# AntreasAntoniou/HowToTrainYourMAMLPytorch

Measured on AMD Instinct MI355X. Metric: meta-tasks/sec, higher is better.
Workload: dtype bf16; 1 GPU; model=maml++_miniimagenet_5w1s, global_batch=128, tasks_per_gpu=128, ways=5, shots=1, targets=15, filters=48, inner_steps=5, msl=True, parallelism=task-dp1

## Files before the change

howtotrainyourmamlpytorch_amd/ops/hip/conv_host.h:

```cpp
#pragma once

#include <cstdlib>
#include <vector>

#include <hip/hip_bf16.h>
#include <torch/extension.h>

namespace maml355 {

inline bool deterministic_mode() {
  const char* e = getenv("MAML355_DETERMINISTIC");
  return e && e[0] == '1';
}

inline int wgrad_nsub_override() {
  const char* e = getenv("MAML355_WGRAD_NSUB");
  return e && (e[0] == '1' || e[0] == '2') ? e[0] - '0' : 0;
}

const __hip_bfloat16* conv_zero_page(const torch::Tensor& like);

std::vector<torch::Tensor> finish_wgrad(const torch::Tensor& acc,
                                        const torch::Tensor& dbacc, int T,
                                        int F, int C, int nslices,
                                        hipStream_t stream);

}
```

howtotrainyourmamlpytorch_amd/ops/hip/tconv.hip:

```cpp

#include "common.h"
#include "conv_host.h"
#include "tconv_mm_addr.h"
#include "wgrad_plan.h"
#include <torch/extension.h>
#include <ATen/cuda/CUDAContext.h>

using namespace maml355;

using bf16 = __hip_bfloat16;
typedef __attribute__((__vector_size__(8 * sizeof(short)))) short bf16x8;
typedef __attribute__((__vector_size__(4 * sizeof(float)))) float f32x4;

DEVINL int swz64(int row, int col) {
  return (row * 64 + col) ^ ((row & 7) << 3);
}
DEVINL int swz128(int row, int col) {
  return (row * 128 + col) ^ ((row & 7) << 3);
}

__global__ void repack_weight_kernel(const float* __restrict__ w,
                                     bf16* __restrict__ wp,
                                     int T, int F, int C, bool dgrad) {
  const long total = (long)T * F * C * 9;
  for (long i = (long)blockIdx.x * blockDim.x + threadIdx.x; i < total;
       i += grid_stride()) {
    long r = i;
    const int kx = (int)(r % 3); r /= 3;
    const int ky = (int)(r % 3); r /= 3;
    const int c = (int)(r % C); r /= C;
    const int f = (int)(r % F); r /= F;
    const long t = r;
    const float v = w[i];
    long o;
    if (!dgrad) {
      o = (((t * 9 + (long)(ky * 3 + kx)) * C + c) * F) + f;
    } else {
      o = (((t * 9 + (long)((2 - ky) * 3 + (2 - kx))) * F + f) * C) + c;
    }
    wp[o] = __float2bfloat16(v);
  }
}

__global__ void wgrad_finalize_kernel(const float* __restrict__ acc,
                                      float* __restrict__ dw,
                                      int T, int F, int C, int nslices) {
  const long total = (long)T * F * C * 9;
  const long ssz = (long)9 * C * F;
  for (long i = (long)blockIdx.x * blockDim.x + threadIdx.x; i < total;
       i += grid_stride()) {
    long r = i;
    const int kx = (int)(r % 3); r /= 3;
    const int ky = (int)(r % 3); r /= 3;
    const int c = (int)(r % C); r /= C;
    const int f = (int)(r % F); r /= F;
    const long t = r;
    const long e = ((long)(ky * 3 + kx) * C + c) * F + f;
    float v = 0.f;
    for (int s = 0; s < nslices; ++s) {
      v += acc[(t * nslices + s) * ssz + e];
    }
    dw[i] = v;
  }
}

#define BM 256
#define BK 64
#define WBK 64

#define WGN 64
static_assert(WBK == wgplan::kStep && WGN == wgplan::kCols,
              "wgrad_plan.h cuts K-chunks for these tiles");

__global__ __launch_bounds__(512, 2)
void tconv_mm_kernel(const bf16* __restrict__ X, const bf16* __restrict__ Wp,
                     const float* __restrict__ bias, bf16* __restrict__ Y,
                     float* __restrict__ sums_out,
                     int T, int NB, int H, int W, int Ci,
                     int Ho, int Wo, int Co, int pad) {
  const int t = blockIdx.y;
  const long Mtot = (long)NB * Ho * Wo;
  const long m0 = (long)blockIdx.x * BM;
  const int K9 = 9 * Ci;
  const int ksteps = (K9 + BK - 1) / BK;
  const int ntiles = (Co + 15) / 16;

  __shared__ short lds_a[BM * BK];
  __shared__ short lds_bt[64 * BK];
  __shared__ int row_h[BM], row_w[BM], row_n[BM];
  __shared__ int ktab_dy[576 + BK], ktab_dx[576 + BK], ktab_c[576 + BK];

  for (int m = threadIdx.x; m < BM; m += blockDim.x) {
    const long mg = m0 + m;
    if (mg < Mtot) {
      const int wo = (int)(mg % Wo);
      const int ho = (int)((mg / Wo) % Ho);
      const int n = (int)(mg / ((long)Wo * Ho));
      row_h[m] = ho; row_w[m] = wo; row_n[m] = n;
    } else {
      row_n[m] = -1;
    }
  }
  for (int k = threadIdx.x; k < ksteps * BK; k += blockDim.x) {
    if (k < K9) {
      const int kyx = k / Ci;
      ktab_c[k] = k - kyx * Ci;
      ktab_dy[k] = kyx / 3;
      ktab_dx[k] = kyx % 3;
    } else {
      ktab_c[k] = -1;
    }
  }

  const bf16* Xt = X + (long)t * NB * H * W * Ci;
  const bf16* Wt = Wp + (long)t * 9 * Ci * Co;

  const int wave = threadIdx.x / WAVE;
  const int lane = threadIdx.x % WAVE;
  const int fr = lane & 15;
  const int fk = lane >> 4;

  f32x4 acc[2][4];
#pragma unroll
  for (int hh = 0; hh < 2; ++hh)
#pragma unroll
    for (int i = 0; i < 4; ++i) acc[hh][i] = {0.f, 0.f, 0.f, 0.f};

  __syncthreads();
  for (int ks = 0; ks < ksteps; ++ks) {
    const int k0 = ks * BK;
    for (int s = threadIdx.x; s < BM * (BK / 8); s += blockDim.x) {
      const int m = s / (BK / 8);
      const int kk0 = (s % (BK / 8)) * 8;
      const int n = row_n[m];
      const int c0 = ktab_c[k0 + kk0];
      const int c7 = ktab_c[k0 + kk0 + 7];
      if ((Ci % 8 == 0) && c0 >= 0 && c7 == c0 + 7) {
        bf16x8 v = {0, 0, 0, 0, 0, 0, 0, 0};
        if (n >= 0) {
          const int h = row_h[m] + ktab_dy[k0 + kk0] - pad;
          const int w = row_w[m] + ktab_dx[k0 + kk0] - pad;
          if (h >= 0 && h < H && w >= 0 && w < W) {
            v = *(const bf16x8*)&(
                (const short*)Xt)[(((long)n * H + h) * W + w) * Ci + c0];
          }
        }
        *(bf16x8*)&lds_a[swz64(m, kk0)] = v;
      } else {
        for (int j = 0; j < 8; ++j) {
          const int kk = kk0 + j;
          const int c = ktab_c[k0 + kk];
          short v = 0;
          if (n >= 0 && c >= 0) {
            const int h = row_h[m] + ktab_dy[k0 + kk] - pad;
            const int w = row_w[m] + ktab_dx[k0 + kk] - pad;
            if (h >= 0 && h < H && w >= 0 && w < W) {
              v = ((const short*)Xt)[(((long)n * H + h) * W + w) * Ci + c];
            }
          }
          lds_a[swz64(m, kk & ~7) + (kk & 7)] = v;
        }
      }
    }
    for (int s = threadIdx.x; s < BK * 8; s += blockDim.x) {
      const int kk = s >> 3;
      const int f0 = (s & 7) * 8;
      if ((Co % 8 == 0) && f0 + 8 <= Co) {
        bf16x8 v = {0, 0, 0, 0, 0, 0, 0, 0};
        if (k0 + kk < K9) {
          v = *(const bf16x8*)&((const short*)Wt)[(long)(k0 + kk) * Co + f0];
        }
#pragma unroll
        for (int j = 0; j < 8; ++j)
          lds_bt[swz64(f0 + j, kk & ~7) + (kk & 7)] = v[j];
      } else {
        for (int j = 0; j < 8 && f0 + j < 64; ++j) {
          const int f = f0 + j;
          short v = 0;
          if (f < Co && k0 + kk < K9) {
            v = ((const short*)Wt)[(long)(k0 + kk) * Co + f];
          }
          lds_bt[swz64(f, kk & ~7) + (kk & 7)] = v;
        }
      }
    }
    __syncthreads();

#pragma unroll
    for (int ksl = 0; ksl < BK / 32; ++ksl) {
      bf16x8 a0 = *(const bf16x8*)&lds_a[swz64(wave * 32 + fr, ksl * 32 + fk * 8)];
      bf16x8 a1 = *(const bf16x8*)&lds_a[swz64(wave * 32 + 16 + fr, ksl * 32 + fk * 8)];
#pragma unroll
      for (int nt = 0; nt < 4; ++nt) {
        if (nt < ntiles) {
          bf16x8 b = *(const bf16x8*)&lds_bt[swz64(nt * 16 + fr, ksl * 32 + fk * 8)];
          acc[0][nt] = __builtin_amdgcn_mfma_f32_16x16x32_bf16(a0, b, acc[0][nt], 0, 0, 0);
          acc[1][nt] = __builtin_amdgcn_mfma_f32_16x16x32_bf16(a1, b, acc[1][nt], 0, 0, 0);
        }
      }
    }
    __syncthreads();
  }

  __shared__ float sums_lds[2][64];
  if (sums_out) {
    for (int i = threadIdx.x; i < 128; i += blockDim.x) {
      sums_lds[i >> 6][i & 63] = 0.f;
    }
    __syncthreads();
  }
  bf16* Yt = Y + (long)t * Mtot * Co;
#pragma unroll
  for (int hh = 0; hh < 2; ++hh)
#pragma unroll
  for (int nt = 0; nt < 4; ++nt) {
    if (nt >= ntiles) break;
    const int col = nt * 16 + fr;
    if (col >= Co) continue;
    const float bv = bias ? bias[(long)t * Co + col] : 0.f;
    float ls = 0.f, lq = 0.f;
#pragma unroll
    for (int j = 0; j < 4; ++j) {
      const int row = wave * 32 + hh * 16 + fk * 4 + j;
      const long mg = m0 + row;
      if (mg < Mtot) {
        const float v = acc[hh][nt][j] + bv;
        ((short*)Yt)[mg * Co + col] =
            (short)__bfloat16_as_short(__float2bfloat16(v));
        ls += v;
        lq += v * v;
      }
    }
    if (sums_out) {
      atomicAdd(&sums_lds[0][col], ls);
      atomicAdd(&sums_lds[1][col], lq);
    }
  }
  if (sums_out) {
    __syncthreads();
    for (int c = threadIdx.x; c < Co; c += blockDim.x) {
      atomicAdd(&sums_out[((long)t * 2 + 0) * Co + c], sums_lds[0][c]);
      atomicAdd(&sums_out[((long)t * 2 + 1) * Co + c], sums_lds[1][c]);
    }
  }
}

#define V2_LDS_BYTES (2 * BM * BK * 2 + 2 * 64 * BK * 2)
#define V2_LDS_BYTES_SBUF (BM * BK * 2 + 64 * BK * 2)

template <bool DBUF>
__global__ __launch_bounds__(512, 2)
void tconv_mm_v2_kernel(const bf16* __restrict__ X, const bf16* __restrict__ Wimg,
                        const float* __restrict__ bias, const bf16* __restrict__ zpage,
                        bf16* __restrict__ Y, float* __restrict__ sums_out,
                        int T, int NB, int H, int W, int Ci,
                        int Ho, int Wo, int Co, int pad) {
  const int t = blockIdx.y;
  const tcmm::Geom g = tcmm::make_geom(NB, H, W, Ci, Ho, Wo, pad);
  const long Mtot = g.Mtot;
  const long m0 = (long)blockIdx.x * BM;
  const int K9 = 9 * Ci;
  const int ksteps = (K9 + BK - 1) / BK;
  const int ntiles = (Co + 15) / 16;

  extern __shared__ short smem[];
#define LDS_A(buf_) (smem + (DBUF ? (buf_) * (BM * BK) : 0))
#define LDS_B(buf_) \
  (smem + (DBUF ? 2 : 1) * (BM * BK) + (DBUF ? (buf_) * (64 * BK) : 0))

  const bf16* Xt = X + (long)t * NB * H * W * Ci;
  const short* Wt = (const short*)Wimg + (long)t * ksteps * 64 * BK;

  const int wave = threadIdx.x / WAVE;
  const int lane = threadIdx.x % WAVE;
  const int fr = lane & 15;
  const int fk = lane >> 4;

  tcmm::KState a_k = tcmm::k_init(g, tcmm::slot_k8(threadIdx.x));
  tcmm::Row a_row[4];
#pragma unroll
  for (int q = 0; q < 4; ++q) {
    a_row[q] = tcmm::row_init(g, m0 + tcmm::slot_row(q * 512 + threadIdx.x));
  }
#define V2_ADVANCE() tcmm::k_advance(g, a_k)

#define V2_STAGE(ks_, buf_)                                                    \
  do {                                                                         \
    _Pragma("unroll")                                                          \
    for (int q = 0; q < 4; ++q) {                                              \
      int off;                                                                 \
      const bf16* src = tcmm::slot_src(g, a_row[q], a_k, off) ? Xt + off       \
                                                              : zpage;         \
      auto ldst = (__attribute__((address_space(3))) void*)(                   \
          &LDS_A(buf_)[((long)q * 512 + wave * 64) * 8]);                      \
      __builtin_amdgcn_global_load_lds(                                        \
          (const __attribute__((address_space(1))) void*)src, ldst, 16, 0, 0); \
    }                                                                          \
    {                                                                          \
      const short* bsrc = Wt + (long)(ks_)*64 * BK + (long)threadIdx.x * 8;    \
      auto ldst = (__attribute__((address_space(3))) void*)(                   \
          &LDS_B(buf_)[(long)wave * 64 * 8]);                                  \
      __builtin_amdgcn_global_load_lds(                                        \
          (const __attribute__((address_space(1))) void*)bsrc, ldst, 16, 0, 0);\
    }                                                                          \
  } while (0)

  f32x4 acc[2][4];
#pragma unroll
  for (int hh = 0; hh < 2; ++hh)
#pragma unroll
    for (int i = 0; i < 4; ++i) acc[hh][i] = {0.f, 0.f, 0.f, 0.f};

  int buf = 0;
  if (DBUF) {
    V2_STAGE(0, 0);
    __syncthreads();
  }
  for (int ks = 0; ks < ksteps; ++ks) {
    if (DBUF) {
      V2_ADVANCE();
      if (ks + 1 < ksteps) V2_STAGE(ks + 1, buf ^ 1);
    } else {
      V2_STAGE(ks, 0);
      V2_ADVANCE();
      __syncthreads();
    }
    const short* la = LDS_A(buf);
    const short* lb = LDS_B(buf);
#pragma unroll
    for (int ksl = 0; ksl < BK / 32; ++ksl) {
      bf16x8 a0 = *(const bf16x8*)&la[swz64(wave * 32 + fr, ksl * 32 + fk * 8)];
      bf16x8 a1 = *(const bf16x8*)&la[swz64(wave * 32 + 16 + fr, ksl * 32 + fk * 8)];
#pragma unroll
      for (int nt = 0; nt < 4; ++nt) {
        if (nt < ntiles) {
          bf16x8 b = *(const bf16x8*)&lb[swz64(nt * 16 + fr, ksl * 32 + fk * 8)];
          acc[0][nt] = __builtin_amdgcn_mfma_f32_16x16x32_bf16(a0, b, acc[0][nt], 0, 0, 0);
          acc[1][nt] = __builtin_amdgcn_mfma_f32_16x16x32_bf16(a1, b, acc[1][nt], 0, 0, 0);
        }
      }
    }
    __syncthreads();
    if (DBUF) buf ^= 1;
  }
#undef V2_STAGE
#undef V2_ADVANCE

  __shared__ float sums_lds[2][64];
  if (sums_out) {
    for (int i = threadIdx.x; i < 128; i += blockDim.x) {
      sums_lds[i >> 6][i & 63] = 0.f;
    }
    __syncthreads();
  }
  bf16* Yt = Y + (long)t * Mtot * Co;
#pragma unroll
  for (int hh = 0; hh < 2; ++hh)
#pragma unroll
  for (int nt = 0; nt < 4; ++nt) {
    if (nt >= ntiles) break;
    const int col = nt * 16 + fr;
    if (col >= Co) continue;
    const float bv = bias ? bias[(long)t * Co + col] : 0.f;
    float ls = 0.f, lq = 0.f;
#pragma unroll
    for (int j = 0; j < 4; ++j) {
      const int row = wave * 32 + hh * 16 + fk * 4 + j;
      const long mg = m0 + row;
      if (mg < Mtot) {
        const float v = acc[hh][nt][j] + bv;
        ((short*)Yt)[mg * Co + col] =
            (short)__bfloat16_as_short(__float2bfloat16(v));
        ls += v;
        lq += v * v;
      }
    }
    if (sums_out) {
      atomicAdd(&sums_lds[0][col], ls);
      atomicAdd(&sums_lds[1][col], lq);
    }
  }
  if (sums_out) {
    __syncthreads();
    for (int c = threadIdx.x; c < Co; c += blockDim.x) {
      atomicAdd(&sums_out[((long)t * 2 + 0) * Co + c], sums_lds[0][c]);
      atomicAdd(&sums_out[((long)t * 2 + 1) * Co + c], sums_lds[1][c]);
    }
  }
}

#undef LDS_A
#undef LDS_B

__global__ void pad_nhwc_kernel(const bf16* __restrict__ x, bf16* __restrict__ xp,
                                int T, int NB, int H, int W, int C, int pad) {
  const int Hp = H + 2 * pad, Wp = W + 2 * pad;
  const int c8n = C / 8;
  const long total = (long)T * NB * Hp * Wp * c8n;
  typedef bf16x8 v8;
  for (long i = (long)blockIdx.x * blockDim.x + threadIdx.x; i < total;
       i += grid_stride()) {
    const int c0 = (int)(i % c8n) * 8;
    long r = i / c8n;
    const int wp = (int)(r % Wp); r /= Wp;
    const int hp = (int)(r % Hp); r /= Hp;
    const long nb = r;
    const int h = hp - pad, w = wp - pad;
    v8 v = {0, 0, 0, 0, 0, 0, 0, 0};
    if (h >= 0 && h < H && w >= 0 && w < W) {
      v = *(const v8*)&((const short*)x)[((nb * H + h) * W + w) * C + c0];
    }
    *(v8*)&((short*)xp)[((nb * Hp + hp) * Wp + wp) * C + c0] = v;
  }
}

__global__ void repack_v2_kernel(const float* __restrict__ w,
                                 bf16* __restrict__ out,
                                 int T, int F, int C, int ksteps, bool dgrad) {
  const int cin = dgrad ? F : C;
  const int cout = dgrad ? C : F;
  const int K9 = 9 * cin;
  const long total = (long)T * ksteps * 64 * BK;
  for (long i = (long)blockIdx.x * blockDim.x + threadIdx.x; i < total;
       i += grid_stride()) {
    const int jj = (int)(i & 7);
    const int j = (int)((i >> 3) & 7);
    const int f = (int)((i >> 6) & 63);
    long r = i >> 12;
    const int ks = (int)(r % ksteps);
    const long t = r / ksteps;
    const int k = ks * BK + ((j ^ (f & 7)) * 8) + jj;
    float v = 0.f;
    if (k < K9 && f < cout) {
      const int kyx = k / cin;
      const int ci = k - kyx * cin;
      const int ky = kyx / 3, kx = kyx % 3;
      if (!dgrad) {
        v = w[((((long)t * F + f) * C + ci) * 3 + ky) * 3 + kx];
      } else {
        v = w[((((long)t * F + ci) * C + f) * 3 + (2 - ky)) * 3 + (2 - kx)];
      }
    }
    out[i] = __float2bfloat16(v);
  }
}


__global__ void dyt_pad_kernel(const bf16* __restrict__ dy,
                               bf16* __restrict__ dyt,
                               int T, int NB, int Ho, int Wo, int F,
                               int Wo8, long Kr) {
  __shared__ short lds[64 * 72];
  long b = blockIdx.x;
  const int ho = (int)(b % Ho); b /= Ho;
  const int n = (int)(b % NB); b /= NB;
  const int t = (int)b;
  const int f8n = (F + 7) / 8;
  const short* src = (const short*)dy + ((((long)t * NB + n) * Ho + ho) * Wo) * F;
  const long k0 = ((long)n * Ho + ho) * Wo8;
  short* dst = (short*)dyt + (long)t * F * Kr + k0;
  for (int wbase = 0; wbase < Wo8; wbase += 64) {
    const int wlen = min(64, Wo8 - wbase);
    for (int s = threadIdx.x; s < wlen * f8n; s += blockDim.x) {
      const int wl = s / f8n;
      const int wo = wbase + wl;
      const int f0 = (s % f8n) * 8;
      bf16x8 v = {0, 0, 0, 0, 0, 0, 0, 0};
      if (wo < Wo && f0 + 8 <= F) {
        v = *(const bf16x8*)&src[(long)wo * F + f0];
      } else if (wo < Wo) {
        for (int j = 0; j < 8 && f0 + j < F; ++j)
          v[j] = src[(long)wo * F + f0 + j];
      }
#pragma unroll
      for (int j = 0; j < 8; ++j) lds[(f0 + j) * 72 + wl] = v[j];
    }
    __syncthreads();
    for (int s = threadIdx.x; s < F * (wlen / 8); s += blockDim.x) {
      const int f = s / (wlen / 8);
      const int w0 = (s % (wlen / 8)) * 8;
      *(bf16x8*)&dst[(long)f * Kr + wbase + w0] =
          *(const bf16x8*)&lds[f * 72 + w0];
    }
    __syncthreads();
  }
}

__global__ void dyt_tail_kernel(bf16* __restrict__ dyt, int T, int F,
                                long Kprime, long Kr) {
  const long tail = Kr - Kprime;
  const long total = (long)T * F * tail;
  for (long i = (long)blockIdx.x * blockDim.x + threadIdx.x; i < total;
       i += grid_stride()) {
    const long c = i % tail;
    const long r = i / tail;
    ((short*)dyt)[r * Kr + Kprime + c] = 0;
  }
}

__global__ void xt_pad_kernel(const bf16* __restrict__ x, bf16* __restrict__ xt,
                              int T, int NB, int H, int W, int C,
                              int Hxp, int Wxp, int pad) {
  __shared__ short lds[64 * 72];
  long b = blockIdx.x;
  const int wt = (int)(b % ((Wxp + 63) / 64)); b /= (Wxp + 63) / 64;
  const int hxp = (int)(b % Hxp); b /= Hxp;
  const int n = (int)(b % NB); b /= NB;
  const int t = (int)b;
  const int h = hxp - pad;
  const int w0 = wt * 64;
  const int c8n = (C + 7) / 8;
  const short* src = (const short*)x + (((long)t * NB + n) * H) * W * C;
  for (int s = threadIdx.x; s < 64 * c8n; s += blockDim.x) {
    const int wl = s / c8n;
    const int c0 = (s % c8n) * 8;
    const int w = w0 + wl - pad;
    bf16x8 v = {0, 0, 0, 0, 0, 0, 0, 0};
    if (h >= 0 && h < H && w >= 0 && w < W) {
      if (c0 + 8 <= C) {
        v = *(const bf16x8*)&src[((long)h * W + w) * C + c0];
      } else {
        for (int j = 0; j < 8 && c0 + j < C; ++j)
          v[j] = src[((long)h * W + w) * C + c0 + j];
      }
    }
#pragma unroll
    for (int j = 0; j < 8; ++j) lds[(c0 + j) * 72 + wl] = v[j];
  }
  __syncthreads();
  short* dst = (short*)xt + ((((long)t * C) * NB + n) * Hxp + hxp) * Wxp;
  for (int s = threadIdx.x; s < C * 8; s += blockDim.x) {
    const int c = s / 8;
    const int wg = (s % 8) * 8;
    const int wx = w0 + wg;
    if (wx + 8 <= Wxp) {
      *(bf16x8*)&dst[((long)c * NB * Hxp) * Wxp + wx] =
          *(const bf16x8*)&lds[c * 72 + wg];
    } else {
      for (int j = 0; j < 8 && wx + j < Wxp; ++j)
        dst[((long)c * NB * Hxp) * Wxp + wx + j] = lds[c * 72 + wg + j];
    }
  }
}

template <int NSUB, bool DET>
__global__ __launch_bounds__(256, 4)
void tconv_wgrad_v2_kernel(const bf16* __restrict__ dYT,
                           const bf16* __restrict__ XT,
                           const bf16* __restrict__ zpage,
                           float* __restrict__ dWacc,
                           float* __restrict__ dBacc,
                           int T, int NB, int Ho, int Wo8, int Hxp, int Wxp,
                           int C, int F, long Kr, long Kprime, int kchunk) {
  const int t = blockIdx.z;
  const int n0 = blockIdx.x * (64 * NSUB);
  const int N9 = 9 * C;
  const long kc0 = (long)blockIdx.y * kchunk;
  const long kc_end = min(kc0 + (long)kchunk, Kr);
  const int mtiles = (F + 15) / 16;
  const long imgS = (long)NB * Hxp * Wxp;

  __shared__ short lds_at[2][64 * WBK];
  __shared__ short lds_bt[2][64 * NSUB * WBK];

  const bf16* dYTt = dYT + (long)t * F * Kr;
  const bf16* XTt = XT + (long)t * C * imgS;

  const int wave = threadIdx.x / WAVE;
  const int lane = threadIdx.x % WAVE;
  const int fr = lane & 15;
  const int fk = lane >> 4;

  int a_f[2], a_k8[2];
#pragma unroll
  for (int q = 0; q < 2; ++q) {
    const int s = q * 256 + threadIdx.x;
    a_f[q] = s >> 3;
    a_k8[q] = ((s & 7) ^ ((s >> 3) & 7)) * 8;
  }
  long b_imgoff[2 * NSUB];
  int b_wo8[2 * NSUB], b_ho[2 * NSUB];
  long b_k[2 * NSUB];
  bool b_valid[2 * NSUB];
#pragma unroll
  for (int q = 0; q < 2 * NSUB; ++q) {
    const int s = q * 256 + threadIdx.x;
    const int n = s >> 3;
    const int ng = n0 + n;
    b_valid[q] = ng < N9;
    const int kyx = b_valid[q] ? ng / C : 0;
    const int c = ng - kyx * C;
    b_k[q] = kc0 + ((s & 7) ^ (n & 7)) * 8;
    const int wo8 = (int)(b_k[q] % Wo8);
    const long line = b_k[q] / Wo8;
    const int ho = (int)(line % Ho);
    const int nimg = (int)(line / Ho);
    b_wo8[q] = wo8;
    b_ho[q] = ho;
    b_imgoff[q] = ((long)c * NB + nimg) * Hxp * Wxp +
                  (long)(ho + kyx / 3) * Wxp + kyx % 3;
  }

#define WG2_STAGE(k0_, buf_)                                                   \
  do {                                                                         \
    _Pragma("unroll")                                                          \
    for (int q = 0; q < 2; ++q) {                                              \
      const bf16* src = (a_f[q] < F)                                           \
                            ? dYTt + (long)a_f[q] * Kr + (k0_) + a_k8[q]       \
                            : zpage;                                           \
      auto ldst = (__attribute__((address_space(3))) void*)(                   \
          &lds_at[buf_][((long)q * 256 + wave * 64) * 8]);                     \
      __builtin_amdgcn_global_load_lds(                                        \
          (const __attribute__((address_space(1))) void*)src, ldst, 16, 0, 0); \
    }                                                                          \
    _Pragma("unroll")                                                          \
    for (int q = 0; q < 2 * NSUB; ++q) {                                       \
      const bf16* src = (b_valid[q] && b_k[q] < Kprime)                        \
                            ? XTt + b_imgoff[q] + b_wo8[q]                     \
                            : zpage;                                           \
      auto ldst = (__attribute__((address_space(3))) void*)(                   \
          &lds_bt[buf_][((long)q * 256 + wave * 64) * 8]);                     \
      __builtin_amdgcn_global_load_lds(                                        \
          (const __attribute__((address_space(1))) void*)src, ldst, 16, 0, 0); \
    }                                                                          \
  } while (0)

#define WG2_ADVANCE()                                                          \
  do {                                                                         \
    _Pragma("unroll")                                                          \
    for (int q = 0; q < 2 * NSUB; ++q) {                                       \
      b_k[q] += WBK;                                                           \
      b_wo8[q] += WBK;                                                         \
      while (b_wo8[q] >= Wo8) {                                                \
        b_wo8[q] -= Wo8;                                                       \
        ++b_ho[q];                                                             \
        b_imgoff[q] += Wxp;                                                    \
        if (b_ho[q] == Ho) {                                                   \
          b_ho[q] = 0;                                                         \
          b_imgoff[q] += (long)(Hxp - Ho) * Wxp;                               \
        }                                                                      \
      }                                                                        \
    }                                                                          \
  } while (0)

  f32x4 acc[NSUB][4];
#pragma unroll
  for (int sb = 0; sb < NSUB; ++sb)
#pragma unroll
// ... 543 lines not shown
```

howtotrainyourmamlpytorch_amd/ops/hip/wgrad_nt.hip:

```cpp

#include "common.h"
#include "conv_host.h"
#include "wgrad_nt_addr.h"
#include "wgrad_plan.h"
#include <torch/extension.h>
#include <ATen/cuda/CUDAContext.h>

using namespace maml355;

using bf16 = __hip_bfloat16;
typedef __attribute__((__vector_size__(8 * sizeof(short)))) short bf16x8;
typedef __attribute__((__vector_size__(4 * sizeof(float)))) float f32x4;
typedef short bf16x4v __attribute__((ext_vector_type(4)));

static_assert(wgnt::kRows == wgplan::kStep,
              "wgrad_plan.h cuts K-chunks for this tile");

enum {
  NT_BIAS_NONE = wgplan::kBiasNone,
  NT_BIAS_ONES = wgplan::kBiasOnes,
  NT_BIAS_COLSUM = wgplan::kBiasColsum
};

__global__ void nt_chpad8_kernel(const bf16* __restrict__ x,
                                 bf16* __restrict__ xp, long M, int C) {
  for (long i = (long)blockIdx.x * blockDim.x + threadIdx.x; i < M;
       i += grid_stride()) {
    bf16x8 v = {0, 0, 0, 0, 0, 0, 0, 0};
    const short* s = (const short*)x + i * C;
#pragma unroll
    for (int j = 0; j < 8; ++j)
      if (j < C) v[j] = s[j];
    *(bf16x8*)((short*)xp + i * 8) = v;
  }
}

DEVINL bf16x4v lds_read_tr(const short* p) {
  return __builtin_amdgcn_ds_read_tr16_b64_v4i16(
      (__attribute__((address_space(3))) bf16x4v*)p);
}

template <int NSUB, int MT, bool DET>
__global__ __launch_bounds__(256, 4)
void tconv_wgrad_nt_kernel(const bf16* __restrict__ dY,
                           const bf16* __restrict__ X,
                           const bf16* __restrict__ zpage,
                           float* __restrict__ dWacc,
                           float* __restrict__ dBacc,
                           wgnt::Geom g, int Cout, long Kr, int kchunk,
                           int bias_mode) {
  const int t = blockIdx.z;
  const int n0 = blockIdx.x * (64 * NSUB);
  const int F = g.F;
  const long kc0 = (long)blockIdx.y * kchunk;
  const long kc_end = min(kc0 + (long)kchunk, Kr);

  __shared__ __attribute__((aligned(16))) short lds_a[2][64 * 64];
  __shared__ __attribute__((aligned(16))) short lds_b[2][NSUB][64 * 64];

  const bf16* dYt = dY + (long)t * g.NB * g.Ho * g.Wo * F;
  const bf16* Xt = X + (long)t * g.NB * g.H * g.W * g.C;

  const int wave = __builtin_amdgcn_readfirstlane(threadIdx.x / WAVE);
  const int lane = threadIdx.x % WAVE;
  const int fr = lane & 15;
  const int fk = lane >> 4;

  int s_ch[2];
  wgnt::Pos s_pos[2];
  long s_k[2];
  wgnt::Col s_col[2][NSUB];
#pragma unroll
  for (int q = 0; q < 2; ++q) {
    const int s = q * 256 + threadIdx.x;
    s_ch[q] = wgnt::slot_chunk(s);
    s_k[q] = kc0 + wgnt::slot_row(s);
    s_pos[q] = wgnt::pos_from_k(g, s_k[q]);
#pragma unroll
    for (int sb = 0; sb < NSUB; ++sb)
      s_col[q][sb] = wgnt::col_from_n(g, n0 + sb * 64 + s_ch[q] * 8);
  }

#define NT_LOAD(src_, dst_)                                                    \
  __builtin_amdgcn_global_load_lds(                                            \
      (const __attribute__((address_space(1))) void*)(src_),                   \
      (__attribute__((address_space(3))) void*)(dst_), 16, 0, 0)

#define NT_STAGE(buf_)                                                         \
  do {                                                                         \
    _Pragma("unroll")                                                          \
    for (int q = 0; q < 2; ++q) {                                              \
      const long ao = wgnt::a_src(g, s_pos[q], s_k[q], s_ch[q]);                         \
      const bf16* asrc = ao == wgnt::kZeroPage ? zpage : dYt + ao;             \
      NT_LOAD(asrc, &lds_a[buf_][(q * 256 + wave * 64) * 8]);                  \
      _Pragma("unroll")                                                        \
      for (int sb = 0; sb < NSUB; ++sb) {                                      \
        const long bo = wgnt::b_src(g, s_pos[q], s_k[q], s_col[q][sb]);        \
        const bf16* bsrc = bo == wgnt::kZeroPage ? zpage : Xt + bo;            \
        NT_LOAD(bsrc, &lds_b[buf_][sb][(q * 256 + wave * 64) * 8]);            \
      }                                                                        \
    }                                                                          \
  } while (0)

#define NT_ADVANCE()                                                           \
  do {                                                                         \
    _Pragma("unroll")                                                          \
    for (int q = 0; q < 2; ++q) {                                              \
      s_k[q] += wgnt::kRows;                                                   \
      wgnt::pos_advance(g, s_pos[q]);                                          \
    }                                                                          \
  } while (0)

  f32x4 acc[NSUB][MT];
#pragma unroll
  for (int sb = 0; sb < NSUB; ++sb)
#pragma unroll
    for (int i = 0; i < MT; ++i) acc[sb][i] = {0.f, 0.f, 0.f, 0.f};

  const int ones_col = (bias_mode == NT_BIAS_ONES) ? g.N9 : -1;
  const int ncols = g.N9 + (bias_mode == NT_BIAS_ONES ? 1 : 0);
  bool sb_active[NSUB], sb_ones[NSUB];
#pragma unroll
  for (int sb = 0; sb < NSUB; ++sb) {
    const int nsub0 = n0 + (sb * 4 + wave) * 16;
    sb_active[sb] = nsub0 < ncols;
    sb_ones[sb] = nsub0 + fr == ones_col;
  }
  const bool do_colsum = (bias_mode == NT_BIAS_COLSUM) && (blockIdx.x == 0);
  float db_acc = 0.f;
  const int db_f = threadIdx.x & 63;
  const int db_q = threadIdx.x >> 6;

  NT_STAGE(0);
  __syncthreads();
  int buf = 0;
  for (long k0 = kc0; k0 < kc_end; k0 += wgnt::kRows) {
    NT_ADVANCE();
    if (k0 + wgnt::kRows < kc_end) NT_STAGE(buf ^ 1);
    const short* la = lds_a[buf];
#pragma unroll
    for (int ks = 0; ks < 2; ++ks) {
      bf16x8 afrag[MT];
#pragma unroll
      for (int mt = 0; mt < MT; ++mt) {
        const bf16x4v a0 = lds_read_tr(la + wgnt::tr_idx(lane, ks, 0, mt));
        const bf16x4v a1 = lds_read_tr(la + wgnt::tr_idx(lane, ks, 1, mt));
        afrag[mt] = {a0[0], a0[1], a0[2], a0[3], a1[0], a1[1], a1[2], a1[3]};
      }
#pragma unroll
      for (int sb = 0; sb < NSUB; ++sb) {
        if (!sb_active[sb]) continue;
        const short* lb = lds_b[buf][sb];
        const bf16x4v b0 = lds_read_tr(lb + wgnt::tr_idx(lane, ks, 0, wave));
        const bf16x4v b1 = lds_read_tr(lb + wgnt::tr_idx(lane, ks, 1, wave));
        bf16x8 bfrag = {b0[0], b0[1], b0[2], b0[3], b1[0], b1[1], b1[2], b1[3]};
        if (sb_ones[sb]) {
          const short one = 0x3F80;
          bfrag = {one, one, one, one, one, one, one, one};
        }
#pragma unroll
        for (int mt = 0; mt < MT; ++mt)
          acc[sb][mt] = __builtin_amdgcn_mfma_f32_16x16x32_bf16(
              afrag[mt], bfrag, acc[sb][mt], 0, 0, 0);
      }
    }
    if (do_colsum && db_f < F) {
#pragma unroll
      for (int kk = db_q * 16; kk < db_q * 16 + 16; ++kk) {
        db_acc += __bfloat162float(__hip_bfloat16(__hip_bfloat16_raw{
            (unsigned short)la[wgnt::lds_idx(kk, db_f)]}));
      }
    }
    __syncthreads();
    buf ^= 1;
  }
#undef NT_STAGE
#undef NT_ADVANCE
#undef NT_LOAD

  if (do_colsum) {
    __shared__ float db_lds[4][64];
    db_lds[db_q][db_f] = db_acc;
    __syncthreads();
    if (db_q == 0 && db_f < F) {
      const float v = db_lds[0][db_f] + db_lds[1][db_f] + db_lds[2][db_f] +
                      db_lds[3][db_f];
      if (DET) {
        dBacc[((long)t * gridDim.y + blockIdx.y) * F + db_f] = v;
      } else {
        atomicAdd(&dBacc[(long)t * F + db_f], v);
      }
    }
  }

  const long sl = DET ? (long)t * gridDim.y + blockIdx.y : (long)t;
  float* dWt = dWacc + sl * 9 * Cout * F;
  float* dBt = dBacc ? dBacc + sl * F : nullptr;
#pragma unroll
  for (int sb = 0; sb < NSUB; ++sb) {
    const int n = n0 + (sb * 4 + wave) * 16 + fr;
    const int orow = wgnt::out_row(g, n, Cout);
    float* dst = nullptr;
    if (orow >= 0) dst = dWt + (long)orow * F;
    else if (n == ones_col) dst = dBt;
    if (dst == nullptr) continue;
#pragma unroll
    for (int mt = 0; mt < MT; ++mt) {
#pragma unroll
      for (int j = 0; j < 4; ++j) {
        const int f = mt * 16 + fk * 4 + j;
        if (f < F) {
          if (DET) {
            dst[f] = acc[sb][mt][j];
          } else {
            atomicAdd(&dst[f], acc[sb][mt][j]);
          }
        }
      }
    }
  }
}

std::vector<torch::Tensor> tconv_wgrad_v3(torch::Tensor dy, torch::Tensor x,
                                          long pad, bool with_bias) {
  TORCH_CHECK(dy.is_cuda() && x.is_cuda());
  TORCH_CHECK(dy.scalar_type() == torch::kBFloat16 &&
              x.scalar_type() == torch::kBFloat16);
  auto dyc = dy.contiguous();
  auto xc = x.contiguous();
  const int T = (int)x.size(0), NB = (int)x.size(1), H = (int)x.size(2),
            W = (int)x.size(3), C = (int)x.size(4);
  const int Ho = (int)dy.size(2), Wo = (int)dy.size(3), F = (int)dy.size(4);
  TORCH_CHECK(F % 8 == 0 && F <= 64, "wgrad_v3 needs F % 8 == 0, F <= 64");
  TORCH_CHECK(C % 8 == 0 || C == 1 || C == 3,
              "wgrad_v3 needs C % 8 == 0 or C in {1, 3}");
  TORCH_CHECK(dy.size(0) == T && dy.size(1) == NB &&
              Ho == H + 2 * pad - 2 && Wo == W + 2 * pad - 2 &&
              Ho >= 1 && Wo >= 1 && pad >= 0 && pad <= 2,
              "wgrad_v3: dy/x shapes do not match a 3x3 stride-1 conv");
  const bool det = deterministic_mode();
  auto stream = at::cuda::getCurrentCUDAStream();

  int Cp = C;
  if (C % 8 != 0) {
    Cp = 8;
    const long M = (long)T * NB * H * W;
    auto xp = torch::empty({T, NB, H, W, 8}, x.options());
    hipLaunchKernelGGL(nt_chpad8_kernel,
                       dim3((unsigned)std::min<long>((M + 255) / 256, 65536)),
                       dim3(256), 0,
                       stream.stream(),
                       reinterpret_cast<const bf16*>(xc.data_ptr()),
                       reinterpret_cast<bf16*>(xp.data_ptr()), M, C);
    xc = xp;
  }
  const char* v2_env = getenv("MAML355_WGRAD_V2");
  const wgplan::Plan p =
      wgplan::v3(T, NB, Ho, Wo, C, with_bias, det,
                 !(v2_env && v2_env[0] == '0'), wgrad_nsub_override());
  const wgnt::Geom g =
      wgnt::make_geom(NB, H, W, Cp, Ho, Wo, F, (int)pad, p.Wk);
  TORCH_CHECK(p.gridy <= 65535 && T <= 65535, "wgrad_v3: grid too large");
  auto fopt = x.options().dtype(torch::kFloat32);
  auto acc = torch::zeros({T, p.nslices, 9 * C, F}, fopt);
  auto dbacc = torch::zeros({T, p.nslices, F}, fopt);
  const bf16* zpage = conv_zero_page(x);
  dim3 grid((unsigned)p.gridx, (unsigned)p.gridy, T);
#define LAUNCH_NT(NS_, MT_, DET_)                                              \
  hipLaunchKernelGGL((tconv_wgrad_nt_kernel<NS_, MT_, DET_>), grid, dim3(256), \
                     0, stream.stream(),                                       \
                     reinterpret_cast<const bf16*>(dyc.data_ptr()),            \
                     reinterpret_cast<const bf16*>(xc.data_ptr()), zpage,      \
                     acc.data_ptr<float>(),                                    \
                     with_bias ? dbacc.data_ptr<float>() : nullptr, g, C,      \
                     p.Kr, p.kchunk, p.bias)
#define LAUNCH_NT_MT(NS_, DET_)                                                \
  switch ((F + 15) / 16) {                                                     \
    case 1: LAUNCH_NT(NS_, 1, DET_); break;                                    \
    case 2: LAUNCH_NT(NS_, 2, DET_); break;                                    \
    case 3: LAUNCH_NT(NS_, 3, DET_); break;                                    \
    default: LAUNCH_NT(NS_, 4, DET_); break;                                   \
  }
  if (p.nsub == 2) {
    if (det) LAUNCH_NT_MT(2, true) else LAUNCH_NT_MT(2, false)
  } else {
    if (det) LAUNCH_NT_MT(1, true) else LAUNCH_NT_MT(1, false)
  }
#undef LAUNCH_NT_MT
#undef LAUNCH_NT
  return finish_wgrad(acc, dbacc, T, F, C, p.nslices, stream.stream());
}
```

Before: 734.3 tasks/s.

## Pipeline LDS DMA with explicit vmcnt waits and single barrier per k-step

Replaces the compiler global_load_lds path with inline-asm LDS DMA that sets m0 explicitly, in both the double-buffered forward conv and the wgrad kernel. Each k-step now waits on vmcnt and takes one barrier at the top instead of two __syncthreads, and the wgrad LDS buffers are merged so the bias reduction scratch reuses buffer space. Launch bounds for NSUB=2 are relaxed to 3 blocks per CU. The aim is less barrier and waitcnt overhead, at the cost of hand-written asm and occupancy/register tradeoffs.

```diff
diff --git a/howtotrainyourmamlpytorch_amd/ops/hip/conv_host.h b/howtotrainyourmamlpytorch_amd/ops/hip/conv_host.h
--- a/howtotrainyourmamlpytorch_amd/ops/hip/conv_host.h
+++ b/howtotrainyourmamlpytorch_amd/ops/hip/conv_host.h
@@ -18,6 +18,11 @@
   return e && (e[0] == '1' || e[0] == '2') ? e[0] - '0' : 0;
 }
 
+inline bool wgrad_pipe_enabled() {
+  const char* e = getenv("MAML355_WGRAD_PIPE");
+  return !(e && e[0] == '0');
+}
+
 const __hip_bfloat16* conv_zero_page(const torch::Tensor& like);
 
 std::vector<torch::Tensor> finish_wgrad(const torch::Tensor& acc,
diff --git a/howtotrainyourmamlpytorch_amd/ops/hip/lds_dma.h b/howtotrainyourmamlpytorch_amd/ops/hip/lds_dma.h
--- /dev/null
+++ b/howtotrainyourmamlpytorch_amd/ops/hip/lds_dma.h
@@ -0,0 +1,38 @@
+#pragma once
+
+#include "common.h"
+
+namespace maml355 {
+
+typedef unsigned lds_ptr;
+
+DEVINL lds_ptr lds_addr(const void* p) {
+  return (lds_ptr)(unsigned long)(__attribute__((address_space(3))) const void*)p;
+}
+
+DEVINL void lds_dma16(const void* gsrc, lds_ptr dst_wave_base) {
+  unsigned keep;
+  const lds_ptr dst = __builtin_amdgcn_readfirstlane(dst_wave_base);
+  asm volatile(
+      "s_mov_b32 %0, m0\n\t"
+      "s_mov_b32 m0, %2\n\t"
+      "s_nop 0\n\t"
+      "global_load_lds_dwordx4 %1, off\n\t"
+      "s_mov_b32 m0, %0"
+      : "=&s"(keep)
+      : "v"(gsrc), "s"(dst)
+      : "memory");
+}
+
+template <int N>
+DEVINL void lds_dma_wait() {
+  asm volatile("s_waitcnt vmcnt(%0)" ::"n"(N) : "memory");
+}
+
+DEVINL void lds_barrier() {
+  asm volatile("s_waitcnt lgkmcnt(0)" ::: "memory");
+  __builtin_amdgcn_s_barrier();
+  asm volatile("" ::: "memory");
+}
+
+}
diff --git a/howtotrainyourmamlpytorch_amd/ops/hip/tconv.hip b/howtotrainyourmamlpytorch_amd/ops/hip/tconv.hip
--- a/howtotrainyourmamlpytorch_amd/ops/hip/tconv.hip
+++ b/howtotrainyourmamlpytorch_amd/ops/hip/tconv.hip
@@ -1,6 +1,7 @@
 
 #include "common.h"
 #include "conv_host.h"
+#include "lds_dma.h"
 #include "tconv_mm_addr.h"
 #include "wgrad_plan.h"
 #include <torch/extension.h>
@@ -284,6 +285,17 @@
   }
 #define V2_ADVANCE() tcmm::k_advance(g, a_k)
 
+#define V2_LOAD(src_, dst_)                                                    \
+  do {                                                                         \
+    if (DBUF) {                                                                \
+      lds_dma16((src_), lds_addr(dst_));                                       \
+    } else {                                                                   \
+      __builtin_amdgcn_global_load_lds(                                        \
+          (const __attribute__((address_space(1))) void*)(src_),               \
+          (__attribute__((address_space(3))) void*)(dst_), 16, 0, 0);          \
+    }                                                                          \
+  } while (0)
+
 #define V2_STAGE(ks_, buf_)                                                    \
   do {                                                                         \
     _Pragma("unroll")                                                          \
@@ -291,17 +303,11 @@
       int off;                                                                 \
       const bf16* src = tcmm::slot_src(g, a_row[q], a_k, off) ? Xt + off       \
                                                               : zpage;         \
-      auto ldst = (__attribute__((address_space(3))) void*)(                   \
-          &LDS_A(buf_)[((long)q * 512 + wave * 64) * 8]);                      \
-      __builtin_amdgcn_global_load_lds(                                        \
-          (const __attribute__((address_space(1))) void*)src, ldst, 16, 0, 0); \
+      V2_LOAD(src, &LDS_A(buf_)[((long)q * 512 + wave * 64) * 8]);             \
     }                                                                          \
     {                                                                          \
       const short* bsrc = Wt + (long)(ks_)*64 * BK + (long)threadIdx.x * 8;    \
-      auto ldst = (__attribute__((address_space(3))) void*)(                   \
-          &LDS_B(buf_)[(long)wave * 64 * 8]);                                  \
-      __builtin_amdgcn_global_load_lds(                                        \
-          (const __attribute__((address_space(1))) void*)bsrc, ldst, 16, 0, 0);\
+      V2_LOAD(bsrc, &LDS_B(buf_)[(long)wave * 64 * 8]);                        \
     }                                                                          \
   } while (0)
 
@@ -312,12 +318,11 @@
     for (int i = 0; i < 4; ++i) acc[hh][i] = {0.f, 0.f, 0.f, 0.f};
 
   int buf = 0;
-  if (DBUF) {
-    V2_STAGE(0, 0);
-    __syncthreads();
-  }
+  if (DBUF) V2_STAGE(0, 0);
   for (int ks = 0; ks < ksteps; ++ks) {
     if (DBUF) {
+      lds_dma_wait<0>();
+      lds_barrier();
       V2_ADVANCE();
       if (ks + 1 < ksteps) V2_STAGE(ks + 1, buf ^ 1);
     } else {
@@ -340,10 +345,11 @@
         }
       }
     }
-    __syncthreads();
     if (DBUF) buf ^= 1;
+    else __syncthreads();
   }
 #undef V2_STAGE
+#undef V2_LOAD
 #undef V2_ADVANCE
 
   __shared__ float sums_lds[2][64];
diff --git a/howtotrainyourmamlpytorch_amd/ops/hip/wgrad_nt.hip b/howtotrainyourmamlpytorch_amd/ops/hip/wgrad_nt.hip
--- a/howtotrainyourmamlpytorch_amd/ops/hip/wgrad_nt.hip
+++ b/howtotrainyourmamlpytorch_amd/ops/hip/wgrad_nt.hip
@@ -1,6 +1,7 @@
 
 #include "common.h"
 #include "conv_host.h"
+#include "lds_dma.h"
 #include "wgrad_nt_addr.h"
 #include "wgrad_plan.h"
 #include <torch/extension.h>
@@ -40,8 +41,8 @@
       (__attribute__((address_space(3))) bf16x4v*)p);
 }
 
-template <int NSUB, int MT, bool DET>
-__global__ __launch_bounds__(256, 4)
+template <int NSUB, int MT, bool DET, bool PIPE>
+__global__ __launch_bounds__(256, NSUB == 2 ? 3 : 4)
 void tconv_wgrad_nt_kernel(const bf16* __restrict__ dY,
                            const bf16* __restrict__ X,
                            const bf16* __restrict__ zpage,
@@ -55,8 +56,10 @@
   const long kc0 = (long)blockIdx.y * kchunk;
   const long kc_end = min(kc0 + (long)kchunk, Kr);
 
-  __shared__ __attribute__((aligned(16))) short lds_a[2][64 * 64];
-  __shared__ __attribute__((aligned(16))) short lds_b[2][NSUB][64 * 64];
+  constexpr int kTile = 64 * 64;
+  constexpr int kBuf = (1 + NSUB) * kTile;
+  __shared__ __attribute__((aligned(16))) short lds[2 * kBuf];
+  float (*db_lds)[64] = (float (*)[64])(lds + 2 * kBuf) - 4;
 
   const bf16* dYt = dY + (long)t * g.NB * g.Ho * g.Wo * F;
   const bf16* Xt = X + (long)t * g.NB * g.H * g.W * g.C;
@@ -82,9 +85,15 @@
   }
 
 #define NT_LOAD(src_, dst_)                                                    \
-  __builtin_amdgcn_global_load_lds(                                            \
-      (const __attribute__((address_space(1))) void*)(src_),                   \
-      (__attribute__((address_space(3))) void*)(dst_), 16, 0, 0)
+  do {                                                                         \
+    if (PIPE) {                                                                \
+      lds_dma16((src_), lds_addr(dst_));                                       \
+    } else {                                                                   \
+      __builtin_amdgcn_global_load_lds(                                        \
+          (const __attribute__((address_space(1))) void*)(src_),               \
+          (__attribute__((address_space(3))) void*)(dst_), 16, 0, 0);          \
+    }                                                                          \
+  } while (0)
 
 #define NT_STAGE(buf_)                                                         \
   do {                                                                         \
@@ -92,12 +101,13 @@
     for (int q = 0; q < 2; ++q) {                                              \
       const long ao = wgnt::a_src(g, s_pos[q], s_k[q], s_ch[q]);                         \
       const bf16* asrc = ao == wgnt::kZeroPage ? zpage : dYt + ao;             \
-      NT_LOAD(asrc, &lds_a[buf_][(q * 256 + wave * 64) * 8]);                  \
+      NT_LOAD(asrc, &lds[(buf_) * kBuf + (q * 256 + wave * 64) * 8]);          \
       _Pragma("unroll")                                                        \
       for (int sb = 0; sb < NSUB; ++sb) {                                      \
         const long bo = wgnt::b_src(g, s_pos[q], s_k[q], s_col[q][sb]);        \
         const bf16* bsrc = bo == wgnt::kZeroPage ? zpage : Xt + bo;            \
-        NT_LOAD(bsrc, &lds_b[buf_][sb][(q * 256 + wave * 64) * 8]);            \
+        NT_LOAD(bsrc, &lds[(buf_) * kBuf + (1 + sb) * kTile +                  \
+                           (q * 256 + wave * 64) * 8]);                        \
       }                                                                        \
     }                                                                          \
   } while (0)
@@ -132,12 +142,16 @@
   const int db_q = threadIdx.x >> 6;
 
   NT_STAGE(0);
-  __syncthreads();
+  if (!PIPE) __syncthreads();
   int buf = 0;
   for (long k0 = kc0; k0 < kc_end; k0 += wgnt::kRows) {
+    if (PIPE) {
+      lds_dma_wait<0>();
+      lds_barrier();
+    }
     NT_ADVANCE();
     if (k0 + wgnt::kRows < kc_end) NT_STAGE(buf ^ 1);
-    const short* la = lds_a[buf];
+    const short* la = lds + buf * kBuf;
 #pragma unroll
     for (int ks = 0; ks < 2; ++ks) {
       bf16x8 afrag[MT];
@@ -150,7 +164,7 @@
 #pragma unroll
       for (int sb = 0; sb < NSUB; ++sb) {
         if (!sb_active[sb]) continue;
-        const short* lb = lds_b[buf][sb];
+        const short* lb = la + (1 + sb) * kTile;
         const bf16x4v b0 = lds_read_tr(lb + wgnt::tr_idx(lane, ks, 0, wave));
         const bf16x4v b1 = lds_read_tr(lb + wgnt::tr_idx(lane, ks, 1, wave));
         bf16x8 bfrag = {b0[0], b0[1], b0[2], b0[3], b1[0], b1[1], b1[2], b1[3]};
@@ -171,15 +185,18 @@
             (unsigned short)la[wgnt::lds_idx(kk, db_f)]}));
       }
     }
-    __syncthreads();
+    if (!PIPE) __syncthreads();
     buf ^= 1;
+  }
+  if (PIPE) {
+    lds_dma_wait<0>();
+    lds_barrier();
   }
 #undef NT_STAGE
 #undef NT_ADVANCE
 #undef NT_LOAD
 
   if (do_colsum) {
-    __shared__ float db_lds[4][64];
     db_lds[db_q][db_f] = db_acc;
     __syncthreads();
     if (db_q == 0 && db_f < F) {
@@ -266,26 +283,29 @@
   auto dbacc = torch::zeros({T, p.nslices, F}, fopt);
   const bf16* zpage = conv_zero_page(x);
   dim3 grid((unsigned)p.gridx, (unsigned)p.gridy, T);
-#define LAUNCH_NT(NS_, MT_, DET_)                                              \
-  hipLaunchKernelGGL((tconv_wgrad_nt_kernel<NS_, MT_, DET_>), grid, dim3(256), \
-                     0, stream.stream(),                                       \
+  const bool pipe = wgrad_pipe_enabled();
+#define LAUNCH_NT(NS_, MT_, DET_, PIPE_)                                       \
+  hipLaunchKernelGGL((tconv_wgrad_nt_kernel<NS_, MT_, DET_, PIPE_>), grid,     \
+                     dim3(256), 0, stream.stream(),                            \
                      reinterpret_cast<const bf16*>(dyc.data_ptr()),            \
                      reinterpret_cast<const bf16*>(xc.data_ptr()), zpage,      \
                      acc.data_ptr<float>(),                                    \
                      with_bias ? dbacc.data_ptr<float>() : nullptr, g, C,      \
                      p.Kr, p.kchunk, p.bias)
-#define LAUNCH_NT_MT(NS_, DET_)                                                \
+#define LAUNCH_NT_MT(NS_, DET_, PIPE_)                                         \
   switch ((F + 15) / 16) {                                                     \
-    case 1: LAUNCH_NT(NS_, 1, DET_); break;                                    \
-    case 2: LAUNCH_NT(NS_, 2, DET_); break;                                    \
-    case 3: LAUNCH_NT(NS_, 3, DET_); break;                                    \
-    default: LAUNCH_NT(NS_, 4, DET_); break;                                   \
-  }
-  if (p.nsub == 2) {
-    if (det) LAUNCH_NT_MT(2, true) else LAUNCH_NT_MT(2, false)
-  } else {
-    if (det) LAUNCH_NT_MT(1, true) else LAUNCH_NT_MT(1, false)
-  }
+    case 1: LAUNCH_NT(NS_, 1, DET_, PIPE_); break;                             \
+    case 2: LAUNCH_NT(NS_, 2, DET_, PIPE_); break;                             \
+    case 3: LAUNCH_NT(NS_, 3, DET_, PIPE_); break;                             \
+    default: LAUNCH_NT(NS_, 4, DET_, PIPE_); break;                            \
+  }
+#define LAUNCH_NT_DET(NS_, PIPE_)                                              \
+  if (det) LAUNCH_NT_MT(NS_, true, PIPE_) else LAUNCH_NT_MT(NS_, false, PIPE_)
+#define LAUNCH_NT_PIPE(NS_)                                                    \
+  if (pipe) { LAUNCH_NT_DET(NS_, true) } else { LAUNCH_NT_DET(NS_, false) }
+  if (p.nsub == 2) { LAUNCH_NT_PIPE(2) } else { LAUNCH_NT_PIPE(1) }
+#undef LAUNCH_NT_PIPE
+#undef LAUNCH_NT_DET
 #undef LAUNCH_NT_MT
 #undef LAUNCH_NT
   return finish_wgrad(acc, dbacc, T, F, C, p.nslices, stream.stream());
```

New measurement: 744.5 tasks/s, median of 6. No clear change (+1.4%).
